# klauspost/compress

Measured on NVIDIA B200. Metric: zstd SpeedFastest encode GB/s (input), higher is better.
Workload: dtype u8

## Files before the change

compress_b200/csrc/b2c_api.cu:

```cuda
#include <cuda_runtime.h>
#include <cstdio>
#include <cstdlib>
#include <cstring>
#include <vector>
#include <thread>
#include <mutex>
#include <condition_variable>
#include <deque>
#include <chrono>
#include <atomic>
#include "../../include/b2c.h"
#include "b2c_zstd_enc.cuh"
#include "b2c_lz.cuh"
#include "b2c_frame.cuh"
#include "b2c_zstd_dec.cuh"
#include "b2c_zstd_dec_staged.cuh"
#include "b2c_s2_dec.cuh"
#include "b2c_s2_stream.cuh"
#include "b2c_huf0.cuh"

#ifndef TABLES_CTAS_PER_SM
#define TABLES_CTAS_PER_SM 8
#endif

// ... 148 lines not shown
    if (cudaGetDeviceCount(&n) != cudaSuccess || n == 0 || device >= n) return nullptr;
    if (cudaSetDevice(device) != cudaSuccess) return nullptr;
    b2c_ctx *ctx = new b2c_ctx();
    ctx->device = device;
    ctx->max_chunks = max_chunks;
    cudaDeviceProp prop;
    if (cudaGetDeviceProperties(&prop, device) != cudaSuccess) { delete ctx; return nullptr; }
    ctx->sm_count = prop.multiProcessorCount;
    bool ok = true;
    {
        size_t a = 0;
        size_t b = (size_t)ctx->sm_count * LzCfg<1>::MIN_CTAS * LzLayout<1>::SCRATCH_BYTES;
        size_t c = (size_t)ctx->sm_count * LzCfg<2>::MIN_CTAS * LzLayout<2>::SCRATCH_BYTES;
        size_t d3 = (size_t)ctx->sm_count * LzCfg<3>::MIN_CTAS * LzLayout<3>::SCRATCH_BYTES;
        size_t d4 = (size_t)ctx->sm_count * LzCfg<4>::MIN_CTAS * LzLayout<4>::SCRATCH_BYTES;
        if (d3 > a) a = d3;
        if (d4 > a) a = d4;
        size_t d5 = (size_t)ctx->sm_count * LzCfg<5>::MIN_CTAS * LzLayout<5>::SCRATCH_BYTES;
        if (d5 > a) a = d5;
        ctx->scratch_slot = ((a > b ? (a > c ? a : c) : (b > c ? b : c)) + 255) & ~(size_t)255;
    }
    ok = ok && cudaMalloc(&ctx->d_scratch, 2 * ctx->scratch_slot) == cudaSuccess;
    ok = ok && cudaEventCreateWithFlags(&ctx->ev_busy, cudaEventDisableTiming) == cudaSuccess;
    ok = ok && cudaFuncSetAttribute(b2c_lz_parse1_kernel, cudaFuncAttributeMaxDynamicSharedMemorySize,
                                    (int)LzLayout<1>::SMEM_BYTES) == cudaSuccess;
    ok = ok && cudaFuncSetAttribute(b2c_lz_parse2_kernel, cudaFuncAttributeMaxDynamicSharedMemorySize,
                                    (int)LzLayout<2>::SMEM_BYTES) == cudaSuccess;
    ok = ok && cudaFuncSetAttribute(b2c_lz_parse3_kernel, cudaFuncAttributeMaxDynamicSharedMemorySize,
                                    (int)LzLayout<5>::SMEM_BYTES) == cudaSuccess;
    ok = ok && cudaFuncSetAttribute(b2c_lz_s2_fast_kernel, cudaFuncAttributeMaxDynamicSharedMemorySize, (int)LzLayout<3>::SMEM_BYTES) == cudaSuccess;
    ok = ok && cudaFuncSetAttribute(b2c_lz_snappy_fast_kernel, cudaFuncAttributeMaxDynamicSharedMemorySize, (int)LzLayout<3>::SMEM_BYTES) == cudaSuccess;
    ok = ok && cudaFuncSetAttribute(b2c_lz_s2_better_kernel, cudaFuncAttributeMaxDynamicSharedMemorySize, (int)LzLayout<4>::SMEM_BYTES) == cudaSuccess;
    ok = ok && cudaFuncSetAttribute(b2c_lz_snappy_better_kernel, cudaFuncAttributeMaxDynamicSharedMemorySize, (int)LzLayout<4>::SMEM_BYTES) == cudaSuccess;
    ok = ok && cudaFuncSetAttribute(b2c_zstd_hist_kernel, cudaFuncAttributeMaxDynamicSharedMemorySize,
                                    (int)HIST_SMEM_BYTES) == cudaSuccess;
    ok = ok && cudaFuncSetAttribute(b2c_zstd_pack128_kernel, cudaFuncAttributeMaxDynamicSharedMemorySize,
                                    (int)PackCfg<131072>::SMEM_BYTES) == cudaSuccess;
    ok = ok && cudaStreamCreateWithFlags(&ctx->stream, cudaStreamNonBlocking) == cudaSuccess;
    ok = ok && cudaFuncSetAttribute(b2c_zstd_chains_kernel, cudaFuncAttributeMaxDynamicSharedMemorySize,
                                    (int)CHAIN_SMEM_BYTES) == cudaSuccess;
    ok = ok && cudaFuncSetAttribute(b2c_huf_compress_kernel, cudaFuncAttributeMaxDynamicSharedMemorySize,
                                    (int)HUF0_SMEM_BYTES) == cudaSuccess;
    ok = ok && cudaFuncSetAttribute(b2c_huf_decompress_kernel, cudaFuncAttributeMaxDynamicSharedMemorySize,
                                    (int)DEC_SMEM_BYTES) == cudaSuccess;
    ok = ok && cudaFuncSetAttribute(b2c_huf_dec_prep_kernel, cudaFuncAttributeMaxDynamicSharedMemorySize,
                                    (int)DEC_SMEM_BYTES) == cudaSuccess;
    ok = ok && cudaFuncSetAttribute(b2c_huf_read_table_kernel, cudaFuncAttributeMaxDynamicSharedMemorySize,
                                    (int)DEC_SMEM_BYTES) == cudaSuccess;
    ok = ok && cudaFuncSetAttribute(b2c_zstd_decode_kernel, cudaFuncAttributeMaxDynamicSharedMemorySize,
                                    (int)DEC_SMEM_BYTES) == cudaSuccess;
    ok = ok && cudaFuncSetAttribute(b2c_zstd_dec_lit_kernel, cudaFuncAttributeMaxDynamicSharedMemorySize,
                                    (int)(FD_LIT_WARPS * FD_LIT_WARP_BYTES)) == cudaSuccess;
    ok = ok && cudaFuncSetAttribute(b2c_zstd_dec_init_kernel, cudaFuncAttributeMaxDynamicSharedMemorySize,
                                    (int)DEC_WARP_BYTES) == cudaSuccess;
    ok = ok && cudaMalloc(&ctx->d_fd_const, FD_CONST_ENTRIES * sizeof(uint32_t)) == cudaSuccess;
    if (ok) {
        b2c_zstd_dec_init_kernel<<<1, 32, DEC_WARP_BYTES>>>(ctx->d_fd_const);
        ok = cudaDeviceSynchronize() == cudaSuccess;
    }
    for (int i = 0; i < 7; i++) ok = ok && cudaEventCreate(&ctx->dec_ev[i]) == cudaSuccess;
    ok = ok && cudaStreamCreateWithFlags(&ctx->dec_aux, cudaStreamNonBlocking) == cudaSuccess;
    ok = ok && cudaEventCreateWithFlags(&ctx->dec_fork, cudaEventDisableTiming) == cudaSuccess;
    ok = ok && cudaEventCreateWithFlags(&ctx->dec_join, cudaEventDisableTiming) == cudaSuccess;
    ok = ok && cudaMalloc(&ctx->d_counters, 256 * sizeof(uint32_t)) == cudaSuccess;
    {
        const char *es = getenv("B2C_ENC_XXH");
        ctx->enc_fused_xxh = (es && strcmp(es, "kernel") == 0) ? 0 : 1;
    }
// ... 228 lines not shown
        }
        P.dbg_cycles = dbg_cycles ? dbg_cycles + (size_t)c0 * 16 * 32 : nullptr;
        cudaEvent_t *pe = nullptr;
        if (ctx->prof) {
            while (ctx->pev.size() < ctx->pev_used + 7) {
                cudaEvent_t e;
                CK(cudaEventCreate(&e));
                ctx->pev.push_back(e);
            }
            pe = ctx->pev.data() + ctx->pev_used;
            ctx->pev_used += 7;
        }
#define PEV(k) do { if (pe) cudaEventRecord(pe[k], st); } while (0)
        PEV(0);
        const bool wantXxh = (flags & B2C_ZSTD_FRAME) && (flags & B2C_ZSTD_CRC);
        if (wantXxh && !ctx->enc_fused_xxh) {
            b2c_zstd_xxh_kernel<<<(4 * m + 127) / 128, 128, 0, st>>>(P);
            ctx->launches += 1;
        }
        { int r = next_counter(ctx, st, &P.counter); if (r) return r; }
        PEV(1);
        {
            if (level == B2C_LEVEL_FASTEST) {
                const unsigned cap = sms * LzCfg<1>::MIN_CTAS, g1 = cap < m ? cap : m;
                b2c_lz_parse1_kernel<<<g1, LzCfg<1>::NT, LzLayout<1>::SMEM_BYTES, st>>>(P);
            } else if (level == B2C_LEVEL_DEFAULT) {
                const unsigned cap = sms * LzCfg<2>::MIN_CTAS, g1 = cap < m ? cap : m;
                b2c_lz_parse2_kernel<<<g1, LzCfg<2>::NT, LzLayout<2>::SMEM_BYTES, st>>>(P);
            } else {
                const unsigned cap = sms * LzCfg<5>::MIN_CTAS, g1 = cap < m ? cap : m;
                b2c_lz_parse3_kernel<<<g1, LzCfg<5>::NT, LzLayout<5>::SMEM_BYTES, st>>>(P);
            }
            PEV(2);
            const unsigned gh = sms * 7 < m ? sms * 7 : m;
            b2c_zstd_hist_kernel<<<gh, HIST_NT, HIST_SMEM_BYTES, st>>>(P);
            ctx->launches += 2;
        }
        PEV(3);
        const unsigned g2 = sms * TABLES_CTAS_PER_SM < m ? sms * TABLES_CTAS_PER_SM : m;
        b2c_zstd_tables_kernel<<<g2, TABLES_NT, 0, st>>>(P);
        PEV(4);
        b2c_zstd_chains_kernel<<<(m + 31) / 32, CHAIN_NT + ((wantXxh && ctx->enc_fused_xxh) ? CHAIN_XXH_NT : 0), CHAIN_SMEM_BYTES, st>>>(P);
        PEV(5);
        if (blockmax > 65536) b2c_zstd_pack128_kernel<<<m, PACK_NT, PackCfg<131072>::SMEM_BYTES, st>>>(P);
        else b2c_zstd_pack_kernel<<<m, PACK_NT, PACK_SMEM_BYTES, st>>>(P);
        PEV(6);
#undef PEV
        ctx->launches += 3;
        CK(cudaGetLastError());
    }
    return ctx_order_end(ctx, st);
}

int b2c_zstd_encode_device(b2c_ctx *ctx, int level, int flags, const void *d_src, size_t src_stride,
                           const uint32_t *d_sizes, uint32_t size_all, void *d_dst, size_t dst_stride,
                           int64_t *d_out_sizes, uint32_t nchunks, void *stream) {
    return launch_encode(ctx, level, flags, d_src, src_stride, d_sizes, size_all, d_dst, dst_stride, d_out_sizes,
                         nchunks, nullptr, nullptr, nullptr, 0, (cudaStream_t)stream);
}

int b2c_zstd_encode_device_debug(b2c_ctx *ctx, int level, int flags, const void *d_src, size_t src_stride,
                                 const uint32_t *d_sizes, uint32_t size_all, void *d_dst, size_t dst_stride,
                                 int64_t *d_out_sizes, uint32_t nchunks, uint32_t *d_dbg_hdr, uint32_t *d_dbg_seqs,
                                 uint8_t *d_dbg_lits, uint32_t dbg_seq_cap, void *stream) {
    return launch_encode(ctx, level, flags, d_src, src_stride, d_sizes, size_all, d_dst, dst_stride,
                         d_out_sizes, nchunks, d_dbg_hdr, d_dbg_seqs, d_dbg_lits, dbg_seq_cap, (cudaStream_t)stream);
}

int b2c_zstd_encode_device_timed(b2c_ctx *ctx, int flags, const void *d_src, size_t src_stride, uint32_t size_all,
// ... 1285 lines not shown
```

compress_b200/csrc/b2c_lz.cuh:

```cuda
#pragma once
#include "b2c_zstd_enc.cuh"

namespace b2c {

constexpr uint32_t LZ_RANGE = 128;
constexpr uint32_t LZ_MAXREC = LZ_RANGE / 4;
constexpr uint32_t LZ_TAGBITS = 14;
constexpr uint32_t LZ_TAGMASK = (1u << LZ_TAGBITS) - 1;
constexpr uint32_t LZ_EMPTY = 0xffffffffu;
#ifndef LZ_PPT1
#define LZ_PPT1 8
#endif
#ifndef LZ_INS_FAST
#define LZ_INS_FAST 2
#endif
constexpr uint32_t LZ_EXT_CAP = 256;

template <int LV> struct LzCfg;
enum { LZ_ZSTD1 = 1, LZ_ZSTD2 = 2, LZ_S2FAST = 3, LZ_S2BETTER = 4, LZ_ZSTD3 = 5 };
template <> struct LzCfg<1> {
    static constexpr int NT = 512;
    static constexpr uint32_t BLOCK = 65536;
    static constexpr bool LONG = false;
    static constexpr int SMLS = 6, LMLS = 8;
// ... 43 lines not shown
    static constexpr uint32_t BLOCK = 65536;
    static constexpr bool LONG = true;
    static constexpr int SMLS = 4, LMLS = 7;
    static constexpr int PPT = 4;
    static constexpr int INS = 1;
    static constexpr uint32_t TBITS = 13;
    static constexpr uint32_t KREC = 12;
    static constexpr int MIN_CTAS = 2;
};

template <int LV> struct LzLayout {
    using C = LzCfg<LV>;
    static constexpr uint32_t NTAB = C::LONG ? 2 : 1;
    static constexpr uint32_t TAB_BYTES = NTAB * (4u << C::TBITS);
    static constexpr uint32_t SRC_BYTES = C::BLOCK + 128;
    static constexpr uint32_t A_BYTES = TAB_BYTES > SRC_BYTES ? TAB_BYTES : SRC_BYTES;
    static constexpr uint32_t BM_BYTES = C::BLOCK / 8 + 16;
    static constexpr uint32_t SM_A = 0;
    static constexpr uint32_t SM_BM = SM_A + A_BYTES;
    static constexpr uint32_t SM_BML = SM_BM + BM_BYTES;
    static constexpr uint32_t SM_REC = SM_BML + (C::LONG ? BM_BYTES : 0);
    static constexpr uint32_t REC_BYTES = C::KREC * C::NT * 4;
    static constexpr uint32_t SM_ARR = SM_REC + REC_BYTES;
    static constexpr uint32_t SM_STG = SM_BM;
    static constexpr uint32_t STG_S2 = ((BM_BYTES * (C::LONG ? 2u : 1u)) / (C::NT / 32)) & ~15u;
    static constexpr uint32_t SM_SH = SM_ARR + C::NT * 14;
    static constexpr uint32_t SMEM_BYTES = SM_SH + ((sizeof(ParseShared) + 2 * 80 * 4 + 15) / 16) * 16;
    static constexpr uint32_t DIST_BYTES = C::BLOCK * 2;
    static constexpr uint32_t SCRATCH_BYTES = DIST_BYTES + (LZ_MAXREC - C::KREC) * C::NT * 4;
};
static_assert(2 * (LzLayout<1>::SMEM_BYTES + 1024) <= 228 * 1024, "two level-1 parse CTAs must fit one SM");
static_assert(LzLayout<2>::SMEM_BYTES <= 227 * 1024 && LzLayout<5>::SMEM_BYTES <= 227 * 1024, "the level-2 / level-3 parse CTA must fit one SM");
static_assert(2 * (LzLayout<3>::SMEM_BYTES + 1024) <= 228 * 1024 && 2 * (LzLayout<4>::SMEM_BYTES + 1024) <= 228 * 1024, "two S2 parse CTAs must fit one SM");

template <int MLS> B2C_DEV uint32_t lz_hash_short(uint32_t lo, uint32_t hi) {
    if constexpr (MLS == 4) return lo * 0x9E3779B1u;
    else if constexpr (MLS == 5) return lo * 0x9E3779B1u + (hi & 0xffu) * 0x85EBCA6Bu;
    else return lo * 0x9E3779B1u + (hi & 0xffffu) * 0x85EBCA6Bu;
}
template <int MLS> B2C_DEV uint32_t lz_hash_long(uint32_t lo, uint32_t hi) {
    if constexpr (MLS == 7) return lo * 0xC2B2AE3Du + (hi & 0xffffffu) * 0x27D4EB2Fu;
    else return lo * 0xC2B2AE3Du + hi * 0x27D4EB2Fu;
}

B2C_DEV void group_scan_excl_pair(uint32_t a, uint32_t b, uint32_t *ws, int nthreads, unsigned tid, uint32_t *exA,
                                  uint32_t *exB, uint32_t *totA, uint32_t *totB) {
    const unsigned lane = tid & 31, w = tid >> 5;
    const uint32_t ia = warp_scan_incl(a), ib = warp_scan_incl(b);
    if (lane == 31) { ws[w] = ia; ws[40 + w] = ib; }
    __syncthreads();
    if (w == 0) {
        const int nw = nthreads >> 5;
        const uint32_t xa = (lane < (unsigned)nw) ? ws[lane] : 0, xb = (lane < (unsigned)nw) ? ws[40 + lane] : 0;
        const uint32_t sa = warp_scan_incl(xa), sb = warp_scan_incl(xb);
        ws[lane] = sa - xa; ws[40 + lane] = sb - xb;
        if (lane == 31) { ws[32] = sa; ws[72] = sb; }
    }
    __syncthreads();
    *exA = ws[w] + ia - a; *exB = ws[40 + w] + ib - b;
    *totA = ws[32]; *totB = ws[72];
}

B2C_DEV uint32_t lz_rec(uint32_t rel, uint32_t len, uint32_t d) { return rel | (len << 7) | (d << 16); }
B2C_DEV uint32_t lz_rec_rel(uint32_t r) { return r & 127u; }
B2C_DEV uint32_t lz_rec_len(uint32_t r) { return (r >> 7) & 511u; }
B2C_DEV uint32_t lz_rec_d(uint32_t r) { return r >> 16; }
// ... 307 lines not shown
        if (cnt) lastE = nextEmit;
    }
    B2C_PHASE(6);
    cntA[tid] = (uint8_t)cnt;
    capA[tid] = (uint8_t)((cnt != 0) && capped);
    longLen[tid] = 0;
    __syncthreads();
    if (w == 0) {
        uint32_t covered = 0;
        for (uint32_t base = 0; base < nlanes; base += 32) {
            const uint32_t t = base + lane;
            unsigned m = __ballot_sync(FULLMASK, t < nlanes && capA[t]);
            while (m) {
                const uint32_t tt = base + (uint32_t)(__ffs((int)m) - 1);
                m &= m - 1;
                const uint32_t r = REC((uint32_t)cntA[tt] - 1, tt);
                const uint32_t s0 = tt * LZ_RANGE + lz_rec_rel(r), l0 = lz_rec_len(r), d0 = lz_rec_d(r);
                const uint32_t e0 = s0 + l0;
                if (e0 > covered) {
                    const uint32_t ext = warp_match_len(src, e0, e0 - d0, n);
                    if (lane == 0) longLen[tt] = l0 + ext;
                    covered = e0 + ext;
                }
            }
        }
    }
    __syncthreads();
    const uint32_t myLong = longLen[tid];
    if (myLong) lastE = b + lz_rec_rel(REC(cnt - 1, tid)) + myLong;
    B2C_PHASE(3);

    uint32_t dummyTotal;
    const uint32_t R = group_scan_excl_max(lastE, sh->ws, 0, NT, tid, &dummyTotal);
    B2C_PHASE(8);
    uint32_t kept = 0, firstKept = cnt, sumLen = 0, keptE = 0, lastOff = 0;
    for (uint32_t j = 0; j < cnt; j++) {
        const uint32_t r = REC(j, tid);
        const uint32_t s0 = b + lz_rec_rel(r), e0 = s0 + ((j + 1 == cnt && myLong) ? myLong : lz_rec_len(r));
        if (e0 <= R) continue;
        const uint32_t s2 = s0 > R ? s0 : R, l2 = e0 - s2;
        if (l2 < 4) continue;
        if (kept == 0) firstKept = j;
        kept++; sumLen += l2; keptE = e0; lastOff = lz_rec_d(r);
    }
    B2C_PHASE(9);
    keptEndA[tid] = keptE;
    lastOffA[tid] = lastOff;
    uint32_t seqEx, lenEx, nseq, sumAll, keyTotal;
    __syncthreads();
    group_scan_excl_pair(kept, sumLen, ws2, NT, tid, &seqEx, &lenEx, &nseq, &sumAll);
    (void)lenEx;
    const uint32_t keyEx = group_scan_excl_max(kept ? tid + 1 : 0u, sh->ws, 0, NT, tid, &keyTotal);
    B2C_PHASE(10);
    const uint32_t nlit = n - hist - sumAll;
    const uint32_t prevE0 = keyEx ? keptEndA[keyEx - 1] : hist;
    const uint32_t pOff0 = keyEx ? lastOffA[keyEx - 1] : 0u;

    if constexpr (!ZSTD) {
        constexpr bool SNAPPY = (MODE == LZ_MODE_SNAPPY);
        const uint32_t hdrLen = n < 128 ? 1u : (n < 16384 ? 2u : 3u);
        const bool firstThread = (seqEx == 0);
        uint32_t mySize = 0;
        {
            uint32_t pe = prevE0, po = pOff0;
            bool fst = firstThread;
            for (uint32_t j = firstKept; j < cnt; j++) {
// ... 138 lines not shown
            const uint32_t incl = warp_scan_incl(kept), excl = incl - kept;
            const uint32_t total = __shfl_sync(FULLMASK, incl, 31);
            const uint32_t gbase = __shfl_sync(FULLMASK, seqEx, 0);
            uint32_t carryE = __shfl_sync(FULLMASK, prevE0, 0), carryD = __shfl_sync(FULLMASK, pOff0, 0);
            for (uint32_t f0 = 0; f0 < total; f0 += 32) {
                const uint32_t f = f0 + lane;
                const bool live = f < total;
                uint32_t o = 0;
#pragma unroll
                for (int st = 16; st > 0; st >>= 1) {
                    const uint32_t c = o + st;
                    const uint32_t v = __shfl_sync(FULLMASK, excl, (int)(c & 31));
                    if (c < 32 && v <= f) o = c;
                }
                const uint32_t oExcl = __shfl_sync(FULLMASK, excl, (int)o), oFirst = __shfl_sync(FULLMASK, firstKept, (int)o);
                const uint32_t oCnt = __shfl_sync(FULLMASK, cnt, (int)o), oLong = __shfl_sync(FULLMASK, myLong, (int)o);
                const uint32_t oR = __shfl_sync(FULLMASK, R, (int)o);
                uint32_t s2 = 0, e0 = 0, d0 = 0;
                if (live) {
                    const uint32_t ot = (tid & ~31u) + o, j = oFirst + (f - oExcl);
                    const uint32_t r = REC(j, ot);
                    const uint32_t s0 = ot * LZ_RANGE + lz_rec_rel(r);
                    e0 = s0 + ((j + 1 == oCnt && oLong) ? oLong : lz_rec_len(r));
                    s2 = s0 > oR ? s0 : oR;
                    d0 = lz_rec_d(r);
                }
                uint32_t pe = __shfl_up_sync(FULLMASK, e0, 1), pd = __shfl_up_sync(FULLMASK, d0, 1);
                if (lane == 0) { pe = carryE; pd = carryD; }
                if (live) {
                    const uint32_t gi = gbase + f, ll = s2 - pe, l2 = e0 - s2;
                    const bool isrep = (gi > 0) && (d0 == pd) && (ll > 0);
                    const uint32_t ofv = isrep ? 1u : d0 + 3;
                    wlen.put(gi, ll, l2 - 3); wof[gi] = ofv;
                    wcodes[TBL_LL * mseq + gi] = (uint8_t)seq_ll_code(ll);
                    wcodes[TBL_OF * mseq + gi] = (uint8_t)highbit32(ofv);
                    wcodes[TBL_ML * mseq + gi] = (uint8_t)seq_ml_code(l2 - 3);
                }
                carryE = __shfl_sync(FULLMASK, e0, 31); carryD = __shfl_sync(FULLMASK, d0, 31);
            }
        }
    }
    B2C_PHASE(11);
    if (tid == 0) { sh->kind = kind; sh->rleLen = 0; }
    __syncthreads();
    if (kind == 0 && nseq == 1 && nlit <= 1 && tid == 0) {
        const uint32_t ll0 = wlen.peek_ll(0), of0 = wof[0];
        if (ll0 == nlit && of0 - 3 == 1) { sh->kind = 2; sh->rleLen = wlen.peek_ml(0) + 3 + ll0; }
        else if (saved < 16) sh->kind = 1;
    } else if (kind == 0 && nseq == 1 && saved < 16 && tid == 0) sh->kind = 1;
    uint32_t litEx, litTotal;
    litEx = group_scan_excl(myLit, sh->ws, 0, NT, tid, &litTotal);
    __syncthreads();
    kind = sh->kind;
    B2C_PHASE(4);

    if (kind == 0) {
        constexpr uint32_t STG = L::REC_BYTES / (NT / 32);
        uint8_t *stg = smem + L::SM_REC + w * STG;
        uint8_t *glit = wk_lit(P, chunk);
        uint32_t gpos = __shfl_sync(FULLMASK, litEx, 0);
        uint32_t ph = (uint32_t)((reinterpret_cast<uintptr_t>(glit) + gpos) & 15), fill = 0;
        const uint32_t nr = (w * 32 * LZ_RANGE >= n) ? 0u : ((n - w * 32 * LZ_RANGE + LZ_RANGE - 1) / LZ_RANGE < 32 ? (n - w * 32 * LZ_RANGE + LZ_RANGE - 1) / LZ_RANGE : 32u);
        for (uint32_t i0 = 0;; i0 += 4) {
            const bool last = i0 >= nr;
            if (last || ph + fill + 512 > STG) {
                lz_warp_flush(stg, ph, fill, glit + gpos, lane);
                gpos += fill; fill = 0;
                ph = (uint32_t)((reinterpret_cast<uintptr_t>(glit) + gpos) & 15);
            }
            if (last) break;
            uint32_t nib[4], pc = 0;
#pragma unroll
            for (int q = 0; q < 4; q++) {
                const uint32_t t = w * 32 + i0 + q;
                const uint32_t mw = (i0 + q < nr) ? mask[4 * t + (lane >> 3)] : 0u;
                nib[q] = (mw >> (4 * (lane & 7))) & 15u;
                pc |= (uint32_t)__popc(nib[q]) << (8 * q);
            }
            const uint32_t incl = warp_scan_incl(pc);
            const uint32_t tots = __shfl_sync(FULLMASK, incl, 31);
            if (tots == 0) continue;
            uint32_t rbase = ph + fill;
#pragma unroll
            for (int q = 0; q < 4; q++) {
                const uint32_t c = (pc >> (8 * q)) & 0xffu;
                if (c) {
                    const uint32_t v = srcw[32 * (w * 32 + i0 + q) + lane];
                    const uint32_t packed = __byte_perm(v, 0u, (uint32_t)plut[nib[q]]);
                    uint8_t *o = stg + rbase + ((incl >> (8 * q)) & 0xffu) - c;
                    o[0] = (uint8_t)packed;
                    if (c > 1) o[1] = (uint8_t)(packed >> 8);
                    if (c > 2) o[2] = (uint8_t)(packed >> 16);
                    if (c > 3) o[3] = (uint8_t)(packed >> 24);
                }
                rbase += (tots >> (8 * q)) & 0xffu;
            }
            fill = rbase - ph;
        }
    }
#undef REC
    if (tid == 0) { W->n = nblk; W->nseq = nseq; W->nlit = nlit; W->kind = kind; W->rleLen = sh->rleLen; }
    __syncthreads();
    B2C_PHASE(5);
    }
}

constexpr int HIST_NT = 128;
constexpr int HIST_WARPS = HIST_NT / 32;
constexpr uint32_t HIST_SLICE = 15u * 16u * HIST_NT;
constexpr uint32_t HIST_SMEM_BYTES = HIST_WARPS * 256 * 32;
template <uint32_t SYMMASK>
B2C_DEV void hist_count_stream(const uint8_t *stream, uint32_t s0, uint32_t s1, uint8_t *col, unsigned tid) {
    const uint4 *s16 = reinterpret_cast<const uint4 *>(stream);
    const uint32_t n16 = (s1 + 15) / 16;
    uint32_t i = s0 / 16 + tid;
    uint4 v = (i < n16) ? B2C_LDG(s16 + i) : make_uint4(0, 0, 0, 0);
    while (i < n16) {
        const uint32_t inext = i + HIST_NT;
        const uint4 vnext = (inext < n16) ? B2C_LDG(s16 + inext) : make_uint4(0, 0, 0, 0);
        const uint32_t wv[4] = {v.x, v.y, v.z, v.w};
#pragma unroll
        for (int k = 0; k < 4; k++) {
            const uint32_t pos = 16 * i + 4 * k;
            if (pos < s1) {
                const uint32_t nv = (pos + 4 <= s1) ? 4u : s1 - pos;
                const uint32_t x = wv[k];
                const uint32_t a0 = x & SYMMASK, a1 = (x >> 8) & SYMMASK, a2 = (x >> 16) & SYMMASK, a3 = (x >> 24) & SYMMASK;
                uint32_t i0 = 1, i1 = nv > 1, i2 = nv > 2, i3 = nv > 3;
                if (a1 == a0) { i0 += i1; i1 = 0; }
                if (a2 == a0) { i0 += i2; i2 = 0; } else if (a2 == a1) { i1 += i2; i2 = 0; }
                if (a3 == a0) { i0 += i3; i3 = 0; } else if (a3 == a1) { i1 += i3; i3 = 0; } else if (a3 == a2) { i2 += i3; i3 = 0; }
                const uint32_t c0 = col[a0 * 32], c1 = col[a1 * 32], c2 = col[a2 * 32], c3 = col[a3 * 32];
                col[a0 * 32] = (uint8_t)(c0 + i0);
                if (i1) col[a1 * 32] = (uint8_t)(c1 + i1);
                if (i2) col[a2 * 32] = (uint8_t)(c2 + i2);
                if (i3) col[a3 * 32] = (uint8_t)(c3 + i3);
            }
        }
        i = inext; v = vnext;
    }
}

B2C_DEV void zstd_hist_chunk(uint8_t *smem, const ZstdEncParams &P, uint32_t chunk) {
    const unsigned tid = threadIdx.x, lane = tid & 31, w = tid >> 5;
    ChunkWork *W = P.work + chunk;
    const uint32_t nlit = W->nlit, nseq = W->nseq;
    const uint8_t *lit = wk_lit(P, chunk);
    if (P.dbg_hdr && W->kind != 3) {
        const WkLens wlen = wk_lens(P, chunk);
        const uint32_t *wof = wk_of(P, chunk);
        for (uint32_t i = tid; i < nseq && i < P.dbg_seq_cap && i < P.maxseq; i += HIST_NT) {
            uint32_t *d = P.dbg_seqs + ((uint64_t)chunk * P.dbg_seq_cap + i) * 3;
            d[0] = wlen.get_ll(i); d[1] = wlen.get_ml(i); d[2] = wof[i];
        }
        if (W->kind == 0)
            for (uint32_t i = tid; i < nlit; i += HIST_NT) P.dbg_lits[(uint64_t)chunk * P.blockmax + i] = lit[i];
    }
    if (W->kind != 0) return;
    uint32_t acc0 = 0, acc1 = 0;
    uint8_t *hcol = smem + w * 256 * 32 + lane;
    for (uint32_t s0 = 0; s0 < nlit; s0 += HIST_SLICE) {
        const uint32_t s1 = (s0 + HIST_SLICE < nlit) ? s0 + HIST_SLICE : nlit;
        for (uint32_t i = tid; i < HIST_SMEM_BYTES / 4; i += HIST_NT) reinterpret_cast<uint32_t *>(smem)[i] = 0;
        __syncthreads();
        hist_count_stream<255>(lit, s0, s1, hcol, tid);
        __syncthreads();
#pragma unroll
        for (int half = 0; half < 2; half++) {
            const uint32_t sym = tid + 128 * half;
            uint32_t c = 0;
#pragma unroll
            for (int k = 0; k < HIST_WARPS; k++) {
                const uint32_t *row = reinterpret_cast<const uint32_t *>(smem + k * 256 * 32 + sym * 32);
#pragma unroll
                for (int j = 0; j < 8; j++) {
                    const uint32_t v = row[(j + (tid >> 2)) & 7];
                    c += (v & 0xff) + ((v >> 8) & 0xff) + ((v >> 16) & 0xff) + (v >> 24);
                }
            }
            if (half == 0) acc0 += c; else acc1 += c;
        }
        __syncthreads();
    }
    W->litHist[tid] = acc0;
    W->litHist[tid + 128] = acc1;
    uint32_t cacc = 0, acc1c = 0;
    const uint8_t *codes = wk_codes(P, chunk, 0);
    const uint32_t mseq = P.maxseq;
    for (uint32_t s0 = 0; s0 < nseq; s0 += HIST_SLICE) {
        const uint32_t s1 = (s0 + HIST_SLICE < nseq) ? s0 + HIST_SLICE : nseq;
        for (uint32_t i = tid; i < HIST_SMEM_BYTES / 4; i += HIST_NT) reinterpret_cast<uint32_t *>(smem)[i] = 0;
        __syncthreads();
#pragma unroll
        for (int c = 0; c < 3; c++) {
            uint8_t *ccol = smem + w * 256 * 32 + c * 64 * 32 + lane;
            hist_count_stream<63>(codes + (uint32_t)c * mseq, s0, s1, ccol, tid);
        }
        __syncthreads();
        for (uint32_t i = tid; i < 192; i += HIST_NT) {
            uint32_t c = 0;
#pragma unroll
            for (int k = 0; k < HIST_WARPS; k++) {
                const uint32_t *row = reinterpret_cast<const uint32_t *>(smem + k * 256 * 32 + i * 32);
#pragma unroll
                for (int jj = 0; jj < 8; jj++) {
                    const uint32_t v = row[(jj + (tid >> 2)) & 7];
                    c += (v & 0xff) + ((v >> 8) & 0xff) + ((v >> 16) & 0xff) + (v >> 24);
                }
            }
            if (i < HIST_NT) cacc += c; else acc1c += c;
        }
        __syncthreads();
    }
    uint32_t *shist = reinterpret_cast<uint32_t *>(smem);
    for (uint32_t i = tid; i < 192; i += HIST_NT) {
        const uint32_t c = (i < HIST_NT) ? cacc : acc1c;
        W->seqHist[i / 64][i % 64] = c;
        const unsigned nz = __ballot_sync(FULLMASK, c != 0);
        if ((i & 31) == 0) shist[i >> 5] = nz;
    }
    __syncthreads();
    if (tid < 3) {
        const uint32_t lo = shist[2 * tid], hi = shist[2 * tid + 1];
        W->maxSym[tid] = hi ? 32 + (31 - (uint32_t)__clz((int)hi)) : (lo ? 31 - (uint32_t)__clz((int)lo) : 0u);
    }
    __syncthreads();
}

#ifndef B2C_EMU
template <int LV, int MODE> B2C_DEV void lz_parse_loop(uint8_t *smem, const ZstdEncParams &P) {
    uint8_t *scratch = P.scratch + (uint64_t)blockIdx.x * LzLayout<LV>::SCRATCH_BYTES;
    ParseShared *sh = reinterpret_cast<ParseShared *>(smem + LzLayout<LV>::SM_SH);
    for (;;) {
        __syncthreads();
        if (threadIdx.x == 0) sh->nextChunk = atomicAdd(P.counter, 1u);
        __syncthreads();
        const uint32_t c = sh->nextChunk;
        if (c >= P.nchunks) break;
        lz_parse_chunk<LV, MODE>(smem, P, c, scratch);
    }
}
#define B2C_LZ_KERNEL(name, LV, MODE)                                                                                      \
    extern "C" __global__ void __launch_bounds__(LzCfg<LV>::NT, LzCfg<LV>::MIN_CTAS) name(ZstdEncParams P) {               \
        extern __shared__ __align__(1024) uint8_t smem[];                                                                  \
        lz_parse_loop<LV, MODE>(smem, P);                                                                                  \
    }
B2C_LZ_KERNEL(b2c_lz_parse1_kernel, 1, LZ_MODE_ZSTD)
B2C_LZ_KERNEL(b2c_lz_parse2_kernel, 2, LZ_MODE_ZSTD)
B2C_LZ_KERNEL(b2c_lz_parse3_kernel, 5, LZ_MODE_ZSTD)
B2C_LZ_KERNEL(b2c_lz_s2_fast_kernel, 3, LZ_MODE_S2)
B2C_LZ_KERNEL(b2c_lz_snappy_fast_kernel, 3, LZ_MODE_SNAPPY)
B2C_LZ_KERNEL(b2c_lz_s2_better_kernel, 4, LZ_MODE_S2)
B2C_LZ_KERNEL(b2c_lz_snappy_better_kernel, 4, LZ_MODE_SNAPPY)
#undef B2C_LZ_KERNEL
extern "C" __global__ void __launch_bounds__(HIST_NT) b2c_zstd_hist_kernel(ZstdEncParams P) {
    extern __shared__ __align__(1024) uint8_t smem[];
    for (uint32_t c = blockIdx.x; c < P.nchunks; c += gridDim.x) zstd_hist_chunk(smem, P, c);
}
#endif

}
```

compress_b200/csrc/b2c_zstd_enc.cuh:

```cuda
#pragma once
#include "b2c_common.cuh"
#include "b2c_fse.cuh"
#include "b2c_huff.cuh"
#include "b2c_seq.cuh"

namespace b2c {

constexpr uint32_t ENC_MAX_CHUNK = 1u << 16;
#ifndef PACK_THREADS
#define PACK_THREADS 512
#endif
#ifndef PACK_SEQ_UNROLL
#define PACK_SEQ_UNROLL 1
#endif
#ifndef PACK_SEQ_COMBINE
#define PACK_SEQ_COMBINE 1
#endif
#ifndef PACK_BITS_LUT
#define PACK_BITS_LUT 1
#endif
#ifndef PACK_MIN_CTAS
#define PACK_MIN_CTAS 2
#endif
constexpr int PACK_UNROLL = PACK_SEQ_UNROLL;
// ... 186 lines not shown
        uint32_t o;
        if (off < 2048) { d[1] = (uint8_t)off; d[0] = (uint8_t)((off >> 8) << 5 | (8 - 4) << 2 | 1); len -= 8; o = 2; }
        else { d[2] = (uint8_t)(off >> 8); d[1] = (uint8_t)off; d[0] = 59 << 2 | 2; len -= 60; o = 3; }
        return o + s2_put_repeat(d + o, off, len);
    }
    if (len >= 12 || off >= 2048) { d[2] = (uint8_t)(off >> 8); d[1] = (uint8_t)off; d[0] = (uint8_t)((len - 1) << 2 | 2); return 3; }
    d[1] = (uint8_t)off; d[0] = (uint8_t)((off >> 8) << 5 | (len - 4) << 2 | 1);
    return 2;
}
B2C_DEV uint32_t snappy_copy_size(uint32_t off, uint32_t len) {
    uint32_t sz = 0;
    while (len > 64) { sz += 3; len -= 60; }
    return sz + ((len >= 12 || off >= 2048) ? 3u : 2u);
}
B2C_DEV uint32_t snappy_put_copy(uint8_t *d, uint32_t off, uint32_t len) {
    uint32_t o = 0;
    while (len > 64) { d[o + 2] = (uint8_t)(off >> 8); d[o + 1] = (uint8_t)off; d[o] = 59 << 2 | 2; len -= 60; o += 3; }
    if (len >= 12 || off >= 2048) { d[o + 2] = (uint8_t)(off >> 8); d[o + 1] = (uint8_t)off; d[o] = (uint8_t)((len - 1) << 2 | 2); return o + 3; }
    d[o + 1] = (uint8_t)off; d[o] = (uint8_t)((off >> 8) << 5 | (len - 4) << 2 | 1);
    return o + 2;
}

#ifndef TABLES_MIN_CTAS
#define TABLES_MIN_CTAS 8
#endif
constexpr int TABLES_NT = 128;
struct TablesShared {
    HufWork hw;
    SeqWork sw;
};
B2C_DEV void zstd_tables_chunk(TablesShared *ts, const ZstdEncParams &P, uint32_t chunk) {
    const unsigned tid = threadIdx.x, lane = tid & 31, w = tid >> 5;
    ChunkWork *W = P.work + chunk;
    if (W->kind != 0) return;
    const uint32_t nseq = W->nseq, nlit = W->nlit;
    if (w == 0) {
        HufWork *hw = &ts->hw;
        for (uint32_t s = lane; s < 256; s += 32) hw->count[s] = W->litHist[s];
        if (lane == 0) { hw->status = HUF_INCOMPRESSIBLE; hw->tableDescLen = 0; hw->tableLog = 0; }
        __syncwarp();
        if (nlit > 16) huf_build_table(hw, nlit, lane, 32, -1);
        __syncwarp();
        if (hw->status == HUF_OK) {
            for (uint32_t s = lane; s < 256; s += 32) { W->ctVal[s] = hw->ctVal[s]; W->ctBits[s] = hw->ctBits[s]; }
            for (uint32_t i = lane; i < hw->tableDescLen; i += 32) W->tableDesc[i] = hw->tableDesc[i];
        }
        if (lane == 0) { W->hufStatus = (uint32_t)hw->status; W->hufTableLog = hw->tableLog; W->tableDescLen = hw->tableDescLen; }
    } else {
        const int which = (int)w - 1;
        SeqWork *sw = &ts->sw;
        for (uint32_t s = lane; s < 64; s += 32) sw->hist[which][s] = W->seqHist[which][s];
        if (lane == 0) sw->maxSym[which] = W->maxSym[which];
        __syncwarp();
        seq_build_table(sw, which, nseq, wk_codes(P, chunk, which)[0], lane);
        __syncwarp();
        const FseCTable *t = seq_table(sw, which);
        const uint32_t *s32 = reinterpret_cast<const uint32_t *>(t);
        uint32_t *d32 = reinterpret_cast<uint32_t *>(&W->tbl[which]);
        for (uint32_t i = lane; i < sizeof(FseCTable) / 4; i += 32) d32[i] = s32[i];
        for (uint32_t i = lane; i < sw->ncountLen[which] && i < 96; i += 32) W->ncount[which][i] = sw->ncount[which][i];
        if (lane == 0) {
            W->mode[which] = sw->mode[which]; W->ncountLen[which] = sw->ncountLen[which];
            if (sw->ncountLen[which] == SEQ_TABLE_ERR) { W->ncountLen[which] = 0; W->kind = 1; }
        }
    }
}

B2C_DEV void zstd_tables_loop(TablesShared *ts, const ZstdEncParams &P, uint32_t first, uint32_t stride) {
// ... 408 lines not shown
```

Measured before the change: 127.8.

## Fuse literal and sequence-code histograms into the LZ parse kernel

```diff
diff --git a/compress_b200/csrc/b2c_api.cu b/compress_b200/csrc/b2c_api.cu
--- a/compress_b200/csrc/b2c_api.cu
+++ b/compress_b200/csrc/b2c_api.cu
@@ -204,8 +204,6 @@
     ok = ok && cudaFuncSetAttribute(b2c_lz_snappy_fast_kernel, cudaFuncAttributeMaxDynamicSharedMemorySize, (int)LzLayout<3>::SMEM_BYTES) == cudaSuccess;
     ok = ok && cudaFuncSetAttribute(b2c_lz_s2_better_kernel, cudaFuncAttributeMaxDynamicSharedMemorySize, (int)LzLayout<4>::SMEM_BYTES) == cudaSuccess;
     ok = ok && cudaFuncSetAttribute(b2c_lz_snappy_better_kernel, cudaFuncAttributeMaxDynamicSharedMemorySize, (int)LzLayout<4>::SMEM_BYTES) == cudaSuccess;
-    ok = ok && cudaFuncSetAttribute(b2c_zstd_hist_kernel, cudaFuncAttributeMaxDynamicSharedMemorySize,
-                                    (int)HIST_SMEM_BYTES) == cudaSuccess;
     ok = ok && cudaFuncSetAttribute(b2c_zstd_pack128_kernel, cudaFuncAttributeMaxDynamicSharedMemorySize,
                                     (int)PackCfg<131072>::SMEM_BYTES) == cudaSuccess;
     ok = ok && cudaStreamCreateWithFlags(&ctx->stream, cudaStreamNonBlocking) == cudaSuccess;
@@ -500,9 +498,7 @@
                 b2c_lz_parse3_kernel<<<g1, LzCfg<5>::NT, LzLayout<5>::SMEM_BYTES, st>>>(P);
             }
             PEV(2);
-            const unsigned gh = sms * 7 < m ? sms * 7 : m;
-            b2c_zstd_hist_kernel<<<gh, HIST_NT, HIST_SMEM_BYTES, st>>>(P);
-            ctx->launches += 2;
+            ctx->launches += 1;
         }
         PEV(3);
         const unsigned g2 = sms * TABLES_CTAS_PER_SM < m ? sms * TABLES_CTAS_PER_SM : m;
diff --git a/compress_b200/csrc/b2c_lz.cuh b/compress_b200/csrc/b2c_lz.cuh
--- a/compress_b200/csrc/b2c_lz.cuh
+++ b/compress_b200/csrc/b2c_lz.cuh
@@ -99,6 +99,9 @@
 static_assert(2 * (LzLayout<1>::SMEM_BYTES + 1024) <= 228 * 1024, "two level-1 parse CTAs must fit one SM");
 static_assert(LzLayout<2>::SMEM_BYTES <= 227 * 1024 && LzLayout<5>::SMEM_BYTES <= 227 * 1024, "the level-2 / level-3 parse CTA must fit one SM");
 static_assert(2 * (LzLayout<3>::SMEM_BYTES + 1024) <= 228 * 1024 && 2 * (LzLayout<4>::SMEM_BYTES + 1024) <= 228 * 1024, "two S2 parse CTAs must fit one SM");
+constexpr uint32_t LZ_HIST_WORDS = 256 + 3 * 64;
+static_assert(LzCfg<1>::NT >= (int)LZ_HIST_WORDS && LzCfg<2>::NT >= (int)LZ_HIST_WORDS && LzCfg<5>::NT >= (int)LZ_HIST_WORDS,
+              "the zstd histograms must fit the longLen array");
 
 template <int MLS> B2C_DEV uint32_t lz_hash_short(uint32_t lo, uint32_t hi) {
     if constexpr (MLS == 4) return lo * 0x9E3779B1u;
@@ -472,6 +475,8 @@
 
     uint32_t dummyTotal;
     const uint32_t R = group_scan_excl_max(lastE, sh->ws, 0, NT, tid, &dummyTotal);
+    uint32_t *const hcnt = longLen;
+    if constexpr (ZSTD) { if (tid < LZ_HIST_WORDS) hcnt[tid] = 0; }
     B2C_PHASE(8);
     uint32_t kept = 0, firstKept = cnt, sumLen = 0, keptE = 0, lastOff = 0;
     for (uint32_t j = 0; j < cnt; j++) {
@@ -676,9 +681,15 @@
                     const bool isrep = (gi > 0) && (d0 == pd) && (ll > 0);
                     const uint32_t ofv = isrep ? 1u : d0 + 3;
                     wlen.put(gi, ll, l2 - 3); wof[gi] = ofv;
-                    wcodes[TBL_LL * mseq + gi] = (uint8_t)seq_ll_code(ll);
-                    wcodes[TBL_OF * mseq + gi] = (uint8_t)highbit32(ofv);
-                    wcodes[TBL_ML * mseq + gi] = (uint8_t)seq_ml_code(l2 - 3);
+                    const uint32_t cll = seq_ll_code(ll), cof = highbit32(ofv), cml = seq_ml_code(l2 - 3);
+                    wcodes[TBL_LL * mseq + gi] = (uint8_t)cll;
+                    wcodes[TBL_OF * mseq + gi] = (uint8_t)cof;
+                    wcodes[TBL_ML * mseq + gi] = (uint8_t)cml;
+                    if (kind == 0) {
+                        atomicAdd(&hcnt[256 + 64 * TBL_LL + cll], 1u);
+                        atomicAdd(&hcnt[256 + 64 * TBL_OF + cof], 1u);
+                        atomicAdd(&hcnt[256 + 64 * TBL_ML + cml], 1u);
+                    }
                 }
                 carryE = __shfl_sync(FULLMASK, e0, 31); carryD = __shfl_sync(FULLMASK, d0, 31);
             }
@@ -733,9 +744,10 @@
                     const uint32_t packed = __byte_perm(v, 0u, (uint32_t)plut[nib[q]]);
                     uint8_t *o = stg + rbase + ((incl >> (8 * q)) & 0xffu) - c;
                     o[0] = (uint8_t)packed;
-                    if (c > 1) o[1] = (uint8_t)(packed >> 8);
-                    if (c > 2) o[2] = (uint8_t)(packed >> 16);
-                    if (c > 3) o[3] = (uint8_t)(packed >> 24);
+                    atomicAdd(&hcnt[packed & 0xffu], 1u);
+                    if (c > 1) { o[1] = (uint8_t)(packed >> 8); atomicAdd(&hcnt[(packed >> 8) & 0xffu], 1u); }
+                    if (c > 2) { o[2] = (uint8_t)(packed >> 16); atomicAdd(&hcnt[(packed >> 16) & 0xffu], 1u); }
+                    if (c > 3) { o[3] = (uint8_t)(packed >> 24); atomicAdd(&hcnt[packed >> 24], 1u); }
                 }
                 rbase += (tots >> (8 * q)) & 0xffu;
             }
@@ -745,131 +757,58 @@
 #undef REC
     if (tid == 0) { W->n = nblk; W->nseq = nseq; W->nlit = nlit; W->kind = kind; W->rleLen = sh->rleLen; }
     __syncthreads();
+    if (kind == 0) {
+        for (uint32_t i = tid; i < 256; i += NT) W->litHist[i] = hcnt[i];
+        if (w < 3) {
+            const uint32_t lo = hcnt[256 + 64 * w + lane], hi = hcnt[256 + 64 * w + 32 + lane];
+            W->seqHist[w][lane] = lo; W->seqHist[w][32 + lane] = hi;
+            const unsigned nzLo = __ballot_sync(FULLMASK, lo != 0), nzHi = __ballot_sync(FULLMASK, hi != 0);
+            if (lane == 0)
+                W->maxSym[w] = nzHi ? 32 + (31 - (uint32_t)__clz((int)nzHi)) : (nzLo ? 31 - (uint32_t)__clz((int)nzLo) : 0u);
+        }
+    }
     B2C_PHASE(5);
     }
 }
 
+#ifdef B2C_EMU
 constexpr int HIST_NT = 128;
-constexpr int HIST_WARPS = HIST_NT / 32;
-constexpr uint32_t HIST_SLICE = 15u * 16u * HIST_NT;
-constexpr uint32_t HIST_SMEM_BYTES = HIST_WARPS * 256 * 32;
-template <uint32_t SYMMASK>
-B2C_DEV void hist_count_stream(const uint8_t *stream, uint32_t s0, uint32_t s1, uint8_t *col, unsigned tid) {
-    const uint4 *s16 = reinterpret_cast<const uint4 *>(stream);
-    const uint32_t n16 = (s1 + 15) / 16;
-    uint32_t i = s0 / 16 + tid;
-    uint4 v = (i < n16) ? B2C_LDG(s16 + i) : make_uint4(0, 0, 0, 0);
-    while (i < n16) {
-        const uint32_t inext = i + HIST_NT;
-        const uint4 vnext = (inext < n16) ? B2C_LDG(s16 + inext) : make_uint4(0, 0, 0, 0);
-        const uint32_t wv[4] = {v.x, v.y, v.z, v.w};
-#pragma unroll
-        for (int k = 0; k < 4; k++) {
-            const uint32_t pos = 16 * i + 4 * k;
-            if (pos < s1) {
-                const uint32_t nv = (pos + 4 <= s1) ? 4u : s1 - pos;
-                const uint32_t x = wv[k];
-                const uint32_t a0 = x & SYMMASK, a1 = (x >> 8) & SYMMASK, a2 = (x >> 16) & SYMMASK, a3 = (x >> 24) & SYMMASK;
-                uint32_t i0 = 1, i1 = nv > 1, i2 = nv > 2, i3 = nv > 3;
-                if (a1 == a0) { i0 += i1; i1 = 0; }
-                if (a2 == a0) { i0 += i2; i2 = 0; } else if (a2 == a1) { i1 += i2; i2 = 0; }
-                if (a3 == a0) { i0 += i3; i3 = 0; } else if (a3 == a1) { i1 += i3; i3 = 0; } else if (a3 == a2) { i2 += i3; i3 = 0; }
-                const uint32_t c0 = col[a0 * 32], c1 = col[a1 * 32], c2 = col[a2 * 32], c3 = col[a3 * 32];
-                col[a0 * 32] = (uint8_t)(c0 + i0);
-                if (i1) col[a1 * 32] = (uint8_t)(c1 + i1);
-                if (i2) col[a2 * 32] = (uint8_t)(c2 + i2);
-                if (i3) col[a3 * 32] = (uint8_t)(c3 + i3);
-            }
-        }
-        i = inext; v = vnext;
-    }
+constexpr uint32_t HIST_SMEM_BYTES = LZ_HIST_WORDS * 4 + 16;
+B2C_DEV void zstd_hist_chunk(uint8_t *smem, const ZstdEncParams &P, uint32_t chunk) {
+    const unsigned tid = threadIdx.x;
+    ChunkWork *W = P.work + chunk;
+    uint32_t *h = reinterpret_cast<uint32_t *>(smem);
+    uint32_t *bad = h + LZ_HIST_WORDS;
+    for (uint32_t i = tid; i < LZ_HIST_WORDS; i += HIST_NT) h[i] = 0;
+    if (tid == 0) *bad = 0;
+    __syncthreads();
+    const bool cand = W->kind == 0;
+    if (cand) {
+        const uint8_t *lit = wk_lit(P, chunk);
+        for (uint32_t i = tid; i < W->nlit; i += HIST_NT) atomicAdd(&h[lit[i]], 1u);
+        for (int t = 0; t < 3; t++) {
+            const uint8_t *codes = wk_codes(P, chunk, t);
+            for (uint32_t i = tid; i < W->nseq; i += HIST_NT) atomicAdd(&h[256 + 64 * t + (codes[i] & 63u)], 1u);
+        }
+    }
+    __syncthreads();
+    if (cand) {
+        for (uint32_t i = tid; i < 256; i += HIST_NT)
+            if (h[i] != W->litHist[i]) *bad = 1;
+        for (uint32_t i = tid; i < 192; i += HIST_NT)
+            if (h[256 + i] != W->seqHist[i / 64][i % 64]) *bad = 1;
+        if (tid < 3) {
+            uint32_t mx = 0;
+            for (uint32_t c = 0; c < 64; c++)
+                if (h[256 + 64 * tid + c]) mx = c;
+            if (mx != W->maxSym[tid]) *bad = 1;
+        }
+    }
+    __syncthreads();
+    if (tid == 0 && *bad) W->kind = 3;
+    __syncthreads();
 }
-
-B2C_DEV void zstd_hist_chunk(uint8_t *smem, const ZstdEncParams &P, uint32_t chunk) {
-    const unsigned tid = threadIdx.x, lane = tid & 31, w = tid >> 5;
-    ChunkWork *W = P.work + chunk;
-    const uint32_t nlit = W->nlit, nseq = W->nseq;
-    const uint8_t *lit = wk_lit(P, chunk);
-    if (P.dbg_hdr && W->kind != 3) {
-        const WkLens wlen = wk_lens(P, chunk);
-        const uint32_t *wof = wk_of(P, chunk);
-        for (uint32_t i = tid; i < nseq && i < P.dbg_seq_cap && i < P.maxseq; i += HIST_NT) {
-            uint32_t *d = P.dbg_seqs + ((uint64_t)chunk * P.dbg_seq_cap + i) * 3;
-            d[0] = wlen.get_ll(i); d[1] = wlen.get_ml(i); d[2] = wof[i];
-        }
-        if (W->kind == 0)
-            for (uint32_t i = tid; i < nlit; i += HIST_NT) P.dbg_lits[(uint64_t)chunk * P.blockmax + i] = lit[i];
-    }
-    if (W->kind != 0) return;
-    uint32_t acc0 = 0, acc1 = 0;
-    uint8_t *hcol = smem + w * 256 * 32 + lane;
-    for (uint32_t s0 = 0; s0 < nlit; s0 += HIST_SLICE) {
-        const uint32_t s1 = (s0 + HIST_SLICE < nlit) ? s0 + HIST_SLICE : nlit;
-        for (uint32_t i = tid; i < HIST_SMEM_BYTES / 4; i += HIST_NT) reinterpret_cast<uint32_t *>(smem)[i] = 0;
-        __syncthreads();
-        hist_count_stream<255>(lit, s0, s1, hcol, tid);
-        __syncthreads();
-#pragma unroll
-        for (int half = 0; half < 2; half++) {
-            const uint32_t sym = tid + 128 * half;
-            uint32_t c = 0;
-#pragma unroll
-            for (int k = 0; k < HIST_WARPS; k++) {
-                const uint32_t *row = reinterpret_cast<const uint32_t *>(smem + k * 256 * 32 + sym * 32);
-#pragma unroll
-                for (int j = 0; j < 8; j++) {
-                    const uint32_t v = row[(j + (tid >> 2)) & 7];
-                    c += (v & 0xff) + ((v >> 8) & 0xff) + ((v >> 16) & 0xff) + (v >> 24);
-                }
-            }
-            if (half == 0) acc0 += c; else acc1 += c;
-        }
-        __syncthreads();
-    }
-    W->litHist[tid] = acc0;
-    W->litHist[tid + 128] = acc1;
-    uint32_t cacc = 0, acc1c = 0;
-    const uint8_t *codes = wk_codes(P, chunk, 0);
-    const uint32_t mseq = P.maxseq;
-    for (uint32_t s0 = 0; s0 < nseq; s0 += HIST_SLICE) {
-        const uint32_t s1 = (s0 + HIST_SLICE < nseq) ? s0 + HIST_SLICE : nseq;
-        for (uint32_t i = tid; i < HIST_SMEM_BYTES / 4; i += HIST_NT) reinterpret_cast<uint32_t *>(smem)[i] = 0;
-        __syncthreads();
-#pragma unroll
-        for (int c = 0; c < 3; c++) {
-            uint8_t *ccol = smem + w * 256 * 32 + c * 64 * 32 + lane;
-            hist_count_stream<63>(codes + (uint32_t)c * mseq, s0, s1, ccol, tid);
-        }
-        __syncthreads();
-        for (uint32_t i = tid; i < 192; i += HIST_NT) {
-            uint32_t c = 0;
-#pragma unroll
-            for (int k = 0; k < HIST_WARPS; k++) {
-                const uint32_t *row = reinterpret_cast<const uint32_t *>(smem + k * 256 * 32 + i * 32);
-#pragma unroll
-                for (int jj = 0; jj < 8; jj++) {
-                    const uint32_t v = row[(jj + (tid >> 2)) & 7];
-                    c += (v & 0xff) + ((v >> 8) & 0xff) + ((v >> 16) & 0xff) + (v >> 24);
-                }
-            }
-            if (i < HIST_NT) cacc += c; else acc1c += c;
-        }
-        __syncthreads();
-    }
-    uint32_t *shist = reinterpret_cast<uint32_t *>(smem);
-    for (uint32_t i = tid; i < 192; i += HIST_NT) {
-        const uint32_t c = (i < HIST_NT) ? cacc : acc1c;
-        W->seqHist[i / 64][i % 64] = c;
-        const unsigned nz = __ballot_sync(FULLMASK, c != 0);
-        if ((i & 31) == 0) shist[i >> 5] = nz;
-    }
-    __syncthreads();
-    if (tid < 3) {
-        const uint32_t lo = shist[2 * tid], hi = shist[2 * tid + 1];
-        W->maxSym[tid] = hi ? 32 + (31 - (uint32_t)__clz((int)hi)) : (lo ? 31 - (uint32_t)__clz((int)lo) : 0u);
-    }
-    __syncthreads();
-}
+#endif
 
 #ifndef B2C_EMU
 template <int LV, int MODE> B2C_DEV void lz_parse_loop(uint8_t *smem, const ZstdEncParams &P) {
@@ -897,10 +836,6 @@
 B2C_LZ_KERNEL(b2c_lz_s2_better_kernel, 4, LZ_MODE_S2)
 B2C_LZ_KERNEL(b2c_lz_snappy_better_kernel, 4, LZ_MODE_SNAPPY)
 #undef B2C_LZ_KERNEL
-extern "C" __global__ void __launch_bounds__(HIST_NT) b2c_zstd_hist_kernel(ZstdEncParams P) {
-    extern __shared__ __align__(1024) uint8_t smem[];
-    for (uint32_t c = blockIdx.x; c < P.nchunks; c += gridDim.x) zstd_hist_chunk(smem, P, c);
+#endif
+
 }
-#endif
-
-}
diff --git a/compress_b200/csrc/b2c_zstd_enc.cuh b/compress_b200/csrc/b2c_zstd_enc.cuh
--- a/compress_b200/csrc/b2c_zstd_enc.cuh
+++ b/compress_b200/csrc/b2c_zstd_enc.cuh
@@ -242,8 +242,21 @@
 B2C_DEV void zstd_tables_chunk(TablesShared *ts, const ZstdEncParams &P, uint32_t chunk) {
     const unsigned tid = threadIdx.x, lane = tid & 31, w = tid >> 5;
     ChunkWork *W = P.work + chunk;
+    const uint32_t nseq = W->nseq, nlit = W->nlit;
+    if (P.dbg_hdr && W->kind != 3) {
+        const WkLens wlen = wk_lens(P, chunk);
+        const uint32_t *wof = wk_of(P, chunk);
+        for (uint32_t i = tid; i < nseq && i < P.dbg_seq_cap && i < P.maxseq; i += TABLES_NT) {
+            uint32_t *d = P.dbg_seqs + ((uint64_t)chunk * P.dbg_seq_cap + i) * 3;
+            d[0] = wlen.get_ll(i); d[1] = wlen.get_ml(i); d[2] = wof[i];
+        }
+        if (W->kind == 0) {
+            const uint8_t *lit = wk_lit(P, chunk);
+            for (uint32_t i = tid; i < nlit; i += TABLES_NT) P.dbg_lits[(uint64_t)chunk * P.blockmax + i] = lit[i];
+        }
+    }
+    if (P.dbg_hdr) __syncthreads();
     if (W->kind != 0) return;
-    const uint32_t nseq = W->nseq, nlit = W->nlit;
     if (w == 0) {
         HufWork *hw = &ts->hw;
         for (uint32_t s = lane; s < 256; s += 32) hw->count[s] = W->litHist[s];
```

Result: faster. 138.8 (median of 6 runs) (+8.6%).
